# tech-srl/code2vec

Measured on NVIDIA H100. Metric: path-contexts/sec (train step, batch 1024x200), higher is better.
Workload: dtype tf32 operands / fp32 accumulate+storage

## Files before the change

### code2vec_b200/csrc/engine.cu

```cuda
#include <cuda_runtime.h>
#include <math.h>
#include <stdio.h>
#include <stdlib.h>
#include <string.h>

#include <string>
#include <utility>
#include <vector>

#include "../../include/c2v_b200.h"
#include "common.cuh"
#include "kernels.cuh"
#include "sgemm.cuh"
#include "umma_gemm.cuh"

using namespace c2v;

namespace {

thread_local std::string g_create_error = "";

constexpr size_t kAlign = 256;
inline size_t align_up(size_t x, size_t a = kAlign) { return (x + a - 1) / a * a; }

// ... 1 lines not shown
constexpr int kSplitDw = 48;

struct Workspace {
  size_t H, Xg, dXg, alpha, v, dv, S, loss_b, lse, loss, part, da_part, lse_part, dl;
  size_t Xg_lo, H_lo, S_lo, tgt_hi, tgt_lo, W_hi, W_lo, v_hi, v_lo;
  size_t WT, WT_lo, vT, vT_lo, tgtT, tgtT_lo;
  size_t true_logit, rscale, v_scaled, slab_flag;
  size_t st_src, st_pth, st_tgt, st_mask, st_target, st_topk_idx, st_topk_val, st_code, st_attn;
  size_t nx_src, nx_pth, nx_tgt;
  size_t sb_src, sb_pth, sb_tgt, sb_mask, sb_target;
  size_t stamp_tok, stamp_path, last_tok, last_path, lr_tab;
  size_t stamp_tgt, last_tgt;
  size_t perm, bkt_count, bkt_cursor, bkt_starts;
  size_t det_keys[2], det_vals[2], det_hist, det_offs, det_starts, det_part;
  size_t samp_stamp, samp_status;
  size_t total;
  size_t ldS;
  size_t ldB;
};

bool dims_ok(const c2v_dims* d, std::string* why) {
  auto bad = [&](const char* m) { if (why) *why = m; return false; };
  if (!d) return bad("dims is NULL");
  if (d->token_vocab < 1 || d->path_vocab < 1 || d->target_vocab < 1) return bad("vocab sizes must be >= 1");
  if (d->embed_dim < 4 || d->embed_dim % 4) return bad("embed_dim must be a positive multiple of 4");
  if (d->code_dim < 4 || d->code_dim % 4 || d->code_dim > 1024) return bad("code_dim must be a multiple of 4 in [4, 1024]");
  if (d->max_contexts < 1) return bad("max_contexts must be >= 1");
  if (d->max_batch < 1) return bad("max_batch must be >= 1");
  if (d->top_k < 1 || d->top_k > 64) return bad("top_k must be in [1, 64]");
  if ((double)d->max_batch * d->max_contexts > 2.0e9) return bad("max_batch * max_contexts overflows int32");
// ... 8 lines not shown
  size_t off = 0;
  auto take = [&](size_t bytes) { size_t o = off; off = align_up(off + bytes); return o; };
  w.H = take(N * D * 4);
  w.Xg = take(N * X * 4);
  w.dXg = take(N * X * 4);
  w.alpha = take(N * 4);
  w.v = take(B * D * 4);
  w.dv = take(B * D * 4);
  w.S = take(B * w.ldS * 4);
  w.loss_b = take(B * 4);
  w.lse = take(B * 4);
  w.true_logit = take(B * 4);
  w.rscale = take(B * 4);
  w.v_scaled = take(B * D * 4);
  w.slab_flag = take(64);
  w.loss = take(64);
  size_t part = (size_t)kSplitDv * B * D;
  if ((size_t)kSplitDw * X * D > part) part = (size_t)kSplitDw * X * D;
  w.part = take(part * 4);
  w.da_part = take(B * D * 4);
  w.lse_part = take(B * (size_t)umma::lse_slots(d.target_vocab) * 8);
  w.dl = take(B * (size_t)(kMaxSampled + 1) * 4);
  w.st_src = take(N * 4);
  w.st_pth = take(N * 4);
  w.st_tgt = take(N * 4);
  w.st_mask = take(N * 4);
  w.nx_src = take(N * 4);
  w.nx_pth = take(N * 4);
  w.nx_tgt = take(N * 4);
  w.st_target = take(B * 4);
// ... 114 lines not shown
  int sort_peer = 1;
  bool bkt_zeroed = false;
  int recompute = 0;
  int exp_slab = 1;
  bool slab_flag_zeroed = false;
  HeadSchedule split_fwd = HEAD_SIMT;
  int gather_occ[2] = {0, 0};
  int adam_epi_prefetch = 0;
  int fuse_sg = 0;
  int fuse_gather = 0;
  int cta_pair = 2;
  int num_sms;
  cudaEvent_t ev_tgt_ready = nullptr;
  int dy_late = 1;
  PendingDy pending_dy;
  cudaStream_t side = nullptr;
  cudaEvent_t ev_fork = nullptr, ev_join = nullptr;
  cudaStream_t copy = nullptr;
  cudaEvent_t ev_h2d[2] = {nullptr, nullptr}, ev_used[2] = {nullptr, nullptr};
  bool used_valid[2] = {false, false};
  uint64_t async_n = 0;
  cudaStream_t side2 = nullptr;
  cudaEvent_t ev_fork2 = nullptr, ev_join2 = nullptr;
  bool dy_in_flight = false;
  bool tgt_armed = false;
  float tgt_lr = 0.f, tgt_b1 = 0.f, tgt_b2 = 0.f, tgt_eps = 0.f;
  int64_t tgt_t = 0;
  int64_t armed_t = 0;
  const int32_t* hint_src = nullptr;
  const int32_t* hint_pth = nullptr;
// ... 679 lines not shown
  else
    C2V_LAUNCH(e, (topk_iter_kernel<<<Bt, kTopkThreads, 0, st>>>(S, e->ws.ldS, Y, k, 0, idx, val, row0)));
  if (stats) C2V_LAUNCH(e, (row_maxsum_kernel<<<Bt, 256, 0, st>>>(nullptr, 0, S, e->ws.ldS, Y, nullptr, 0, row_max, row_sum, nullptr)));
  return C2V_OK;
}

int run_dy(c2v_engine* e, cudaStream_t st, const float* v, int B, const SlabDesc& slab);

int run_pending_dy(c2v_engine* e, cudaStream_t st) {
  if (!e->pending_dy.v) return C2V_OK;
  const PendingDy p = e->pending_dy;
  e->pending_dy = PendingDy{};
  return run_dy(e, st, p.v, p.B, p.slab);
}

int context_backward(c2v_engine* e, cudaStream_t st, const ContextSource& cs, const float* mask, int B,
                     const Dropout& dp, const float* dv) {
  const int D = e->dims.code_dim, d = e->dims.embed_dim, K3 = 3 * d, N = cs.rows;
  float* H = wsp<float>(e, e->ws.H);
  float* alpha = wsp<float>(e, e->ws.alpha);
  float* da_part = wsp<float>(e, e->ws.da_part);
  float* part = wsp<float>(e, e->ws.part);
  int rc;
  if (ordered_route(e) && e->inbox.world < 2)
    return fail(e, C2V_ERR_STATE, "ordered_exchange: the gradient rows of row-sharded tables travel through the scatter inbox, "
                                  "and none is bound (c2v_bind_scatter_inbox)");
  if (!is_tc(e) && (rc = run_pending_dy(e, st))) return rc;
  const bool x3 = is_tc(e) && is_3x(e);
  float* H_lo = x3 ? wsp<float>(e, e->ws.H_lo) : nullptr;
  rc = launch_attn_bwd(e, st, H, alpha, dv, wsp<float>(e, e->ws.v), B, da_part, H_lo);
  if (rc) return rc;
  rc = launch_colsum(e, st, da_part, (size_t)D, B, D, e->grad.a);
  if (rc) return rc;
  if (is_tc(e)) {
    float* Xg = wsp<float>(e, e->ws.Xg);
    float* dXg = wsp<float>(e, e->ws.dXg);
    {
      PhaseTimer pt(e, PH_DX_GEMM, st);
      umma::Operand opA{H, (size_t)D, false, H_lo};
      umma::Operand opB{x3 ? wsp<float>(e, e->ws.W_hi) : e->theta.W, (size_t)D, false, x3 ? wsp<float>(e, e->ws.W_lo) : nullptr};
      umma::EpiStore ep{dXg, (size_t)K3, 0};
      C2V_LAUNCH(e, C2V_CUDA(e, (umma::launch(st, N, K3, D, 1, opA, opB, ep, e->num_sms))));
    }
    if (e->lazy) {
      if (e->lazy_grads_pending)
        return fail(e, C2V_ERR_STATE, "lazy_adam: every train step must be followed by c2v_adam_step before the next one");
      e->lazy_grads_pending = true;
    } else if (!e->emb_grads_clean && e->table_world == 1) {
      C2V_CUDA(e, cudaMemsetAsync(e->grad.tok, 0, (size_t)e->dims.token_vocab * d * 4, st));
      C2V_CUDA(e, cudaMemsetAsync(e->grad.path, 0, (size_t)e->dims.path_vocab * d * 4, st));
    }
    C2V_CUDA(e, cudaEventRecord(e->ev_fork, st));
    C2V_CUDA(e, cudaStreamWaitEvent(e->side, e->ev_fork, 0));
    {
      PhaseTimer pt(e, PH_DX_SCATTER, e->side);
      BucketPlan bp;
      if (ordered_route(e)) {
        e->sorted_src = nullptr;
        if ((rc = exchange_scatter(e, e->side, cs, mask, dp, dXg, false))) return rc;
      } else if (e->inbox.world > 1 && plan_buckets(e, &bp, true)) {
        if (e->sorted_src != cs.src || e->sorted_rows != cs.rows) {
          if ((rc = sort_entries(e, e->side, cs, bp))) return rc;
        }
        e->sorted_src = nullptr;
        const int32_t* starts = wsp<int32_t>(e, e->ws.bkt_starts);
        C2V_LAUNCH(e, (inbox_counts_kernel<<<1, 32, 0, e->side>>>(e->inbox, bp, starts)));
        C2V_LAUNCH(e, (scatter_inbox_kernel<<<(3 * N + 7) / 8, 256, 0, e->side>>>(cs, dp, mask, wsp<int32_t>(e, e->ws.perm), starts, bp, dXg,
                                                                              e->inbox, e->grad_scale)));
      } else if (plan_buckets(e, &bp)) {
        if ((rc = sort_entries(e, e->side, cs, bp))) return rc;
        C2V_LAUNCH(e, (scatter_sorted_kernel<<<(3 * N + 7) / 8, 256, 0, e->side>>>(cs, dp, mask, wsp<int32_t>(e, e->ws.perm), dXg, e->gr_tok,
                                                                               e->gr_path, e->grad_scale)));
      } else if (e->deterministic) {
        if ((rc = det_scatter(e, e->side, cs, mask, dp, dXg, false))) return rc;
      } else {
        C2V_LAUNCH(e, (scatter_dx_kernel<<<(N + 7) / 8, 256, 0, e->side>>>(cs, dp, mask, dXg, e->gr_tok, e->gr_path, e->grad_scale)));
      }
    }
    if ((rc = early_catchup(e, e->side))) return rc;
    C2V_CUDA(e, cudaEventRecord(e->ev_join, e->side));
    if ((rc = run_pending_dy(e, st))) return rc;
    {
      PhaseTimer pt(e, PH_DW, st);
      umma::Operand opA{Xg, (size_t)K3, true, x3 ? wsp<float>(e, e->ws.Xg_lo) : nullptr};
      umma::Operand opB{H, (size_t)D, true, H_lo};
      const int ks = umma::effective_splits(N, kSplitDw);
      umma::EpiStore ep{part, (size_t)D, (size_t)K3 * D};
      C2V_LAUNCH(e, C2V_CUDA(e, (umma::launch(st, K3, D, N, kSplitDw, opA, opB, ep, e->num_sms))));
      rc = launch_colsum(e, st, part, (size_t)K3 * D, ks, K3 * D, e->grad.W);
      if (rc) return rc;
    }
    C2V_CUDA(e, cudaStreamWaitEvent(st, e->ev_join, 0));
    if (e->dy_in_flight) {
      C2V_CUDA(e, cudaStreamWaitEvent(st, e->ev_join2, 0));
      e->dy_in_flight = false;
    }
    e->emb_grads_clean = false;
    return C2V_OK;
  }
  {
    PhaseTimer pt(e, PH_DW, st);
    simt::GatherColsX al{cs, dp};
    simt::ColsX bl{H, (size_t)D};
    const int ks = simt::effective_ksplit(N, kSplitDw);
    simt::StoreC ep{part, (size_t)D, (size_t)K3 * D};
    C2V_LAUNCH(e, C2V_CUDA(e, simt::launch(st, K3, D, N, kSplitDw, al, bl, ep)));
    rc = launch_colsum(e, st, part, (size_t)K3 * D, ks, K3 * D, e->grad.W);
// ... 239 lines not shown
      if ((rc = slab_to_p(e, st, hs, v, B, g, &slab, &v_dy))) return rc;
      C2V_LAUNCH(e, (loss_reduce_kernel<<<1, 256, 0, st>>>(loss_b, B, invB, loss_out)));
    }
  } else {
    if ((rc = run_logits(e, st, v, B, hs == HEAD_SIMT ? LOGITS_STORE : LOGITS_STORE_LSE, {}, true))) return rc;
    PhaseTimer pt(e, PH_XENT, st);
    if (hs == HEAD_SIMT) {
      C2V_LAUNCH(e, (xent_kernel<<<B, kXentThreads, 0, st>>>(S, e->ws.ldS, target, Y, invB, loss_b, lse, 1)));
    } else {
      C2V_LAUNCH(e, (xent_combine_kernel<<<B, 256, 0, st>>>(part, n_tiles, S, e->ws.ldS, target, loss_b, lse)));
      if ((rc = slab_to_p(e, st, hs, v, B, g, &slab, &v_dy))) return rc;
    }
    C2V_LAUNCH(e, (loss_reduce_kernel<<<1, 256, 0, st>>>(loss_b, B, invB, loss_out)));
  }
  if ((rc = target_grad_gemms(e, st, v_dy, B, dv, slab))) return rc;
  return context_backward(e, st, cs, mask, B, dp, dv);
}

int sampled_train_step_impl(c2v_engine* e, cudaStream_t st, const int32_t* src, const int32_t* pth, const int32_t* tgt,
                             const float* mask, const int32_t* target, int B, const int32_t* sampled, int S,
                             const float* logq_true, const float* logq_samp, float keep, uint64_t seed, uint64_t step,
                             const float* ext_mask, float* loss_out) {
  if (!e->has_grad) return fail(e, C2V_ERR_STATE, "gradients not bound (c2v_bind_grads)");
  if (!(keep > 0.f) || keep > 1.f) return fail(e, C2V_ERR_INVALID, "keep_prob must be in (0, 1]");
  if (S < 1 || S > kMaxSampled) return fail(e, C2V_ERR_INVALID, "number of sampled classes must be in [1, 1024]");
  const int D = e->dims.code_dim;
  const Dropout dp = make_dropout(e->dims, keep, seed, step, ext_mask);
  ContextSource cs = make_source(e, src, pth, tgt, B);
  float* H = wsp<float>(e, e->ws.H);
  float* alpha = wsp<float>(e, e->ws.alpha);
  float* v = wsp<float>(e, e->ws.v);
// ... 270 lines not shown
    if (value && !exchange_keys_fit(e->dims))
      return fail(e, C2V_ERR_UNSUPPORTED, "ordered_exchange: the padded rows of both tables over all ranks must be below 2^31");
    e->ordered_exchange = (int)value;
    return C2V_OK;
  }
  if (!strcmp(key, "profile")) { e->profile = value ? 1 : 0; return C2V_OK; }
  if (!strcmp(key, "dy_late")) {
    if (value < 0 || value > 2) return fail(e, C2V_ERR_INVALID, "dy_late must be 0, 1 or 2");
    e->dy_late = (int)value;
    return C2V_OK;
  }
  if (!strcmp(key, "fuse_target_adam")) { e->fuse_tgt = value ? 1 : 0; return C2V_OK; }
  if (!strcmp(key, "fuse_gather")) { e->fuse_gather = value ? 1 : 0; return C2V_OK; }
  if (!strcmp(key, "fuse_softmax_grad")) { e->fuse_sg = value ? 1 : 0; return C2V_OK; }
  if (!strcmp(key, "exp_slab")) { e->exp_slab = value ? 1 : 0; return C2V_OK; }
  if (!strcmp(key, "adam_epilogue_prefetch")) { e->adam_epi_prefetch = value ? 1 : 0; return C2V_OK; }
  if (!strcmp(key, "recompute_logits")) { e->recompute = value ? 1 : 0; return C2V_OK; }
  if (!strcmp(key, "sort_peer_access")) {
    if (value < 0 || value > 2) return fail(e, C2V_ERR_INVALID, "sort_peer_access must be 0 (never), 1 (auto) or 2 (always)");
    e->sort_peer = (int)value;
    return C2V_OK;
  }
  if (!strcmp(key, "adam_rest_shortcut")) { e->rest_shortcut = value ? 1 : 0; return C2V_OK; }
  if (!strcmp(key, "adam_sweep_period")) {
    if (value < 0 || value > kLrRing / 2) return fail(e, C2V_ERR_INVALID, "adam_sweep_period must be in [0, 32768]");
    e->sweep_period = (int)value;
    return C2V_OK;
  }
  if (!strcmp(key, "adam_rows_occupancy")) {
    if (value != 4 && value != 5) return fail(e, C2V_ERR_INVALID, "adam_rows_occupancy must be 4 or 5");
// ... 80 lines not shown
        return C2V_ERR_CUDA;
      *value = n;
    }
    return C2V_OK;
  }
  if (!strcmp(key, "profile")) { *value = e->profile; return C2V_OK; }
  if (!strcmp(key, "lazy_adam")) { *value = e->lazy; return C2V_OK; }
  if (!strcmp(key, "adam_sweep_period")) { *value = e->sweep_period; return C2V_OK; }
  if (!strcmp(key, "adam_rest_shortcut")) { *value = e->rest_shortcut; return C2V_OK; }
  if (!strcmp(key, "cta_pair")) { *value = e->cta_pair; return C2V_OK; }
  if (!strcmp(key, "dy_late")) { *value = e->dy_late; return C2V_OK; }
  if (!strcmp(key, "fuse_target_adam")) { *value = e->fuse_tgt; return C2V_OK; }
  if (!strcmp(key, "fuse_gather")) { *value = e->fuse_gather; return C2V_OK; }
  if (!strcmp(key, "fuse_softmax_grad")) { *value = e->fuse_sg; return C2V_OK; }
  if (!strcmp(key, "exp_slab")) { *value = e->exp_slab; return C2V_OK; }
  if (!strcmp(key, "adam_epilogue_prefetch")) { *value = e->adam_epi_prefetch; return C2V_OK; }
  if (!strcmp(key, "exp_slab_fallbacks")) {
    *value = 0;
    if (e->wbase && e->slab_flag_zeroed) {
      unsigned n = 0;
      if (cudaDeviceSynchronize() != cudaSuccess ||
          cudaMemcpy(&n, e->wbase + e->ws.slab_flag + 4, 4, cudaMemcpyDeviceToHost) != cudaSuccess)
        return C2V_ERR_CUDA;
      *value = n;
    }
    return C2V_OK;
  }
  if (!strcmp(key, "sampler_cap_hits")) {
    *value = 0;
    if (e->wbase && e->sample_tag) {
// ... 602 lines not shown
  if (!ordered_route(e)) return fail(e, C2V_ERR_STATE, "set ordered_exchange and bind row-sharded tables over more than one rank first");
  if (e->inbox.world < 2) return fail(e, C2V_ERR_STATE, "no scatter inbox bound (c2v_bind_scatter_inbox)");
  if ((int64_t)n_tok + n_path > 3ll * e->dims.max_batch * e->dims.max_contexts)
    return fail(e, C2V_ERR_INVALID, "n_tok + n_path must be at most 3 * max_batch * max_contexts");
  if (((uintptr_t)tok_vals | (uintptr_t)path_vals) % 16) return fail(e, C2V_ERR_INVALID, "tok_vals and path_vals must be 16-byte aligned");
  C2V_CUDA(e, cudaSetDevice(e->device));
  cudaStream_t st = (cudaStream_t)stream;
  const size_t d = (size_t)e->dims.embed_dim;
  float* vals = wsp<float>(e, e->ws.dXg);
  if (n_tok) C2V_CUDA(e, cudaMemcpyAsync(vals, tok_vals, n_tok * d * 4, cudaMemcpyDeviceToDevice, st));
  if (n_path) C2V_CUDA(e, cudaMemcpyAsync(vals + n_tok * d, path_vals, n_path * d * 4, cudaMemcpyDeviceToDevice, st));
  return exchange_push(e, st, ExchangeListKeys{tok_rows, path_rows, n_tok, exchange_key_map(e)}, n_tok + n_path,
                       DetListContrib{vals, (int)d});
}

int64_t c2v_launch_count(const c2v_engine* e) { return e ? e->launches : 0; }

int c2v_phase_count(void) { return PH_COUNT; }

const char* c2v_phase_name(int phase) { return (phase >= 0 && phase < PH_COUNT) ? kPhaseNames[phase] : ""; }

int c2v_phase_stats(c2v_engine* e, int phase, double* total_ms, int64_t* count, int reset) {
  if (!e || phase < 0 || phase >= PH_COUNT) return C2V_ERR_INVALID;
  C2V_CUDA(e, cudaSetDevice(e->device));
  PhaseLog& L = e->phase[phase];
  if (!L.pending.empty()) C2V_CUDA(e, cudaDeviceSynchronize());
  for (auto& ev : L.pending) {
    float ms = 0.f;
    if (cudaEventElapsedTime(&ms, ev.first, ev.second) == cudaSuccess) { L.total_ms += ms; L.count++; }
    L.free_list.push_back(ev);
// ... 10 lines not shown
```

### code2vec_b200/csrc/kernels.cuh

```cuda
#pragma once
#include <float.h>
#include <limits.h>
#include "common.cuh"

namespace c2v {

constexpr int kAttnThreads = 128;
constexpr int kAttnWarps = kAttnThreads / 32;

__device__ __forceinline__ float block_sum(float v, float* red) {
  const int lane = threadIdx.x & 31, warp = threadIdx.x >> 5, nw = (blockDim.x + 31) >> 5;
  v = warp_sum(v);
  __syncthreads();
  if (lane == 0) red[warp] = v;
  __syncthreads();
  float r = (threadIdx.x < nw) ? red[threadIdx.x] : 0.f;
  if (warp == 0) {
    r = warp_sum(r);
    if (lane == 0) red[0] = r;
  }
  __syncthreads();
  r = red[0];
  __syncthreads();
  return r;
// ... 917 lines not shown
  if (mask[n] == 0.f) return;
  const int K3 = 3 * cs.d;
  const float* src = dXg + (size_t)n * K3;
  for (int j = lane * 4; j < K3; j += 128) {
    float4 g = *reinterpret_cast<const float4*>(src + j);
    const float4 m = dropout_mult4(dp, n, j >> 2);
    g.x *= m.x * grad_scale; g.y *= m.y * grad_scale; g.z *= m.z * grad_scale; g.w *= m.w * grad_scale;
    const int seg = j / cs.d, off = j - seg * cs.d;
    float* dst;
    if (seg == 0) dst = table_row(g_tok, cs.src[n], cs.d) + off;
    else if (seg == 1) dst = table_row(g_path, cs.pth[n], cs.d) + off;
    else dst = table_row(g_tok, cs.tgt[n], cs.d) + off;
    atomicAdd(reinterpret_cast<float4*>(dst), g);
  }
}

constexpr int kMaxBuckets = 8192;

struct BucketPlan {
  int shift, mask;
  int page_shift;
  int pages_tok, pages_path;
  int n_buckets;
};
__device__ __forceinline__ int bucket_of(const BucketPlan& bp, int seg, int idx) {
  const int owner = idx & bp.mask, page = (idx >> bp.shift) >> bp.page_shift;
  return (seg == 1) ? (bp.mask + 1) * bp.pages_tok + owner * bp.pages_path + page : owner * bp.pages_tok + page;
}
__device__ __forceinline__ int entry_index(const ContextSource& cs, int e) {
  const int n = e / 3, seg = e - 3 * n;
// ... 722 lines not shown
```

### code2vec_b200/csrc/umma_gemm.cuh

```cuda
#pragma once
#include <cuda.h>
#include <cuda_runtime.h>
#include <limits.h>
#include <stdint.h>

#include "common.cuh"

namespace c2v {
namespace umma {

constexpr int BM = 128;
constexpr int BN = 128;
constexpr int BK = 32;
constexpr int WG_K = 8;
constexpr int STAGES = 4;
constexpr int kThreads = 4 * 128;
constexpr int kRegsProducer = 72;
constexpr int kRegsConsumer = 128;
constexpr int kRegsEpilogue = 184;
static_assert(kRegsProducer + 2 * kRegsConsumer + kRegsEpilogue == 4 * 128, "the roles share the CTA's registers");

__device__ __forceinline__ float fast_tanh(float x) {
  float e, r;
  asm("ex2.approx.ftz.f32 %0, %1;" : "=f"(e) : "f"(x * 2.885390081777927f));
// ... 8 lines not shown
}
__device__ __forceinline__ void mbar_expect_tx(uint64_t* bar, uint32_t bytes) {
  asm volatile("mbarrier.expect_tx.relaxed.cta.shared::cta.b64 [%0], %1;" ::"r"(smem_u32(bar)), "r"(bytes) : "memory");
}
__device__ __forceinline__ void mbar_arrive(uint64_t* bar) {
  asm volatile("mbarrier.arrive.shared::cta.b64 _, [%0];" ::"r"(smem_u32(bar)) : "memory");
}
__device__ __forceinline__ void mbar_arrive_expect_tx(uint64_t* bar, uint32_t bytes) {
  asm volatile("mbarrier.arrive.expect_tx.shared::cta.b64 _, [%0], %1;" ::"r"(smem_u32(bar)), "r"(bytes) : "memory");
}
__device__ __forceinline__ bool mbar_try_wait(uint64_t* bar, uint32_t parity) {
  uint32_t ok;
  asm volatile(
      "{\n\t.reg .pred p;\n\t"
      "mbarrier.try_wait.parity.shared::cta.b64 p, [%1], %2;\n\t"
      "selp.u32 %0, 1, 0, p;\n\t}"
      : "=r"(ok) : "r"(smem_u32(bar)), "r"(parity) : "memory");
  return ok != 0;
}
template <bool SLEEP = false>
__device__ __forceinline__ void mbar_wait(uint64_t* bar, uint32_t parity) {
  if (mbar_try_wait(bar, parity)) return;
  const long long t0 = clock64();
  uint32_t ns = 32;
  while (!mbar_try_wait(bar, parity)) {
    if (SLEEP) {
      __nanosleep(ns);
      if (ns < 256) ns *= 2;
    }
    if (clock64() - t0 > 20000000000LL) __trap();
// ... 611 lines not shown
  size_t lda;
};

struct SmemLayout {
  static constexpr int kABytes = BM * BK * 4;
  static constexpr int kBBytes = BN * BK * 4;
  static constexpr int kStageBytes = kABytes + kBBytes;
  static constexpr int kEpiOffset = STAGES * kStageBytes;
  static constexpr int kEpiBytes = 64 * BN * 4;
  static constexpr int kBarOffset = kEpiOffset + 2 * kEpiBytes;
  static constexpr int kTotal = kBarOffset + 256 + 1024;
  static_assert((3 * STAGES + 2) * 8 <= 256, "the barriers fit their block");
  static_assert(kTotal <= 232448, "exceeds the 227 KB of shared memory a CTA can opt into");
};

template <bool A_MN, bool B_MN, class Epi, class AX = AXNone, bool B_T = false>
__global__ void __launch_bounds__(kThreads, 1)
umma_gemm_kernel(const __grid_constant__ CUtensorMap tmA, const __grid_constant__ CUtensorMap tmB,
                 const __grid_constant__ CUtensorMap tmAlo, const __grid_constant__ CUtensorMap tmBlo, GemmShape gs,
                 GemmPtrs ptr, Epi epi, AX ax = AX{}, BTransposed bt = {}) {
  if (epi_gate_closed(epi, 0)) return;
  using L = SmemLayout;
  static_assert(!(A_MN && AX::kKind == 2), "the gathered A tile is K-major");
  constexpr bool kTmaA = !A_MN && AX::kKind == 0;
  constexpr bool kTmaB = !B_MN;
  static_assert(!B_T || (kTmaA && kTmaB), "the B tile is copied out of all-K-major TMA stages");
  constexpr uint32_t kTxBytes = (kTmaA ? L::kABytes : 0) + (kTmaB ? L::kBBytes : 0);
  constexpr uint32_t kMnTxBytes = (A_MN ? L::kABytes : 0) + (B_MN ? L::kBBytes : 0);
  constexpr int kLag = kMnTxBytes ? STAGES - 2 : 0;
  static_assert(kLag <= STAGES - 2, "the producer would wait for a stage only a step it has not published can free");
  extern __shared__ uint8_t smem_raw[];
  uint8_t* smem = reinterpret_cast<uint8_t*>((reinterpret_cast<uintptr_t>(smem_raw) + 1023) & ~(uintptr_t)1023);
  uint64_t* full_bar = reinterpret_cast<uint64_t*>(smem + L::kBarOffset);
  uint64_t* empty_bar = full_bar + STAGES;
  uint64_t* landed_bar = empty_bar + STAGES;
// ... 174 lines not shown
    if constexpr (epi_move_regs<Epi>(0)) wg_regs_inc<kRegsEpilogue>();
    const int w = warp & 3;
    float* stg = reinterpret_cast<float*>(smem + L::kEpiOffset + (w >> 1) * L::kEpiBytes);
    auto prefetch_item = [&](int it) {
      if (it >= total_items) return;
      int mt2, nt2, sp2;
      decode(it, mt2, nt2, sp2);
      epi_prefetch_tile(epi, mt2 * BM + 32 * w + lane, nt2 * BN, BN, gs.M, gs.N, 0);
    };
    prefetch_item(blockIdx.x);
    uint32_t epi_phase = 0;
    for (int item = blockIdx.x; item < total_items; item += gridDim.x, epi_phase ^= 1) {
      int mt, nt, sp;
      decode(item, mt, nt, sp);
      prefetch_item(item + gridDim.x);
      mbar_wait<true>(epi_full, epi_phase);
      const int m_base = mt * BM + 32 * w, m = m_base + lane;
      float* cbase = epi.out(sp);
#pragma unroll 1
      for (int p = 0; p < 2; ++p) {
        typename Epi::State est;
        epi.begin(est);
#pragma unroll 1
        for (int q = p; q < 4; q += 2) {
          float* blk = stg + ((w & 1) | (q << 1)) * 1024;
          uint32_t r[32];
#pragma unroll
          for (int c4 = 0; c4 < 8; ++c4) {
            const float4 x = *reinterpret_cast<const float4*>(blk + lane * 32 + ((c4 ^ (lane & 7)) << 2));
            r[4 * c4] = __float_as_uint(x.x); r[4 * c4 + 1] = __float_as_uint(x.y);
            r[4 * c4 + 2] = __float_as_uint(x.z); r[4 * c4 + 3] = __float_as_uint(x.w);
          }
          __syncwarp();
          const int n = nt * BN + 32 * q;
          if (n < gs.N) {
            if (m < gs.M) epi.observe(m, n, r, gs.N - n, est);
            if (epi_stores<Epi>(0)) store_chunk(epi, est, r, blk, lane, m_base, n, gs.M, gs.N, cbase, epi.ldc);
          }
        }
        epi.end(m, 2 * nt + p, sp, m < gs.M, est);
      }
      mbar_arrive(epi_empty);
    }
  }
}

typedef CUresult (*EncodeTiledFn)(CUtensorMap*, CUtensorMapDataType, cuuint32_t, void*, const cuuint64_t*, const cuuint64_t*,
                                  const cuuint32_t*, const cuuint32_t*, CUtensorMapInterleave, CUtensorMapSwizzle,
                                  CUtensorMapL2promotion, CUtensorMapFloatOOBfill);

inline EncodeTiledFn get_encode_fn() {
  static EncodeTiledFn fn = nullptr;
  if (!fn) {
    void* p = nullptr;
    cudaDriverEntryPointQueryResult qres;
    if (cudaGetDriverEntryPoint("cuTensorMapEncodeTiled", &p, cudaEnableDefault, &qres) == cudaSuccess && p)
      fn = reinterpret_cast<EncodeTiledFn>(p);
// ... 50 lines not shown
inline GemmShape make_shape(int M, int N, int K, int splits, int terms) {
  GemmShape gs;
  gs.M = M; gs.N = N; gs.K = K;
  gs.terms = terms;
  gs.m_tiles = (M + BM - 1) / BM;
  gs.n_tiles = (N + BN - 1) / BN;
  const int total_kblocks = (K + BK - 1) / BK;
  if (splits < 1) splits = 1;
  if (splits > total_kblocks) splits = total_kblocks;
  gs.kblocks_per_split = (total_kblocks + splits - 1) / splits;
  gs.splits = (total_kblocks + gs.kblocks_per_split - 1) / gs.kblocks_per_split;
  gs.n_fastest = (gs.n_tiles < gs.m_tiles) ? 1 : 0;
  return gs;
}

template <bool A_MN, bool B_MN, class Epi, class AX, bool B_T = false>
inline cudaError_t launch_kernel(cudaStream_t st, const CUtensorMap& tmA, const CUtensorMap& tmB, const CUtensorMap& tmAlo,
                                 const CUtensorMap& tmBlo, const GemmShape& gs, const GemmPtrs& ptr, const Epi& epi, int num_sms,
                                 const AX& ax, const BTransposed& bt = {}) {
  auto kern = umma_gemm_kernel<A_MN, B_MN, Epi, AX, B_T>;
  cudaError_t e = cudaFuncSetAttribute(kern, cudaFuncAttributeMaxDynamicSharedMemorySize, SmemLayout::kTotal);
  if (e != cudaSuccess) return e;
  int grid = gs.m_tiles * gs.n_tiles * gs.splits;
  if (grid > num_sms) grid = num_sms;
  kern<<<grid, kThreads, SmemLayout::kTotal, st>>>(tmA, tmB, tmAlo, tmBlo, gs, ptr, epi, ax, bt);
  return cudaGetLastError();
}

template <bool A_MN, bool B_MN, class Epi, class AX = AXNone, bool B_T = false>
inline cudaError_t launch_cfg(cudaStream_t st, int M, int N, int K, int splits, const Operand& A, const Operand& B, const Epi& epi,
                              int num_sms, const AX& ax = AX{}, const BTransposed& bt = {}) {
  CUtensorMap tmA{}, tmB{}, tmAlo{}, tmBlo{};
  const bool three = A.lo != nullptr && B.lo != nullptr;
  if ((A.lo != nullptr) != (B.lo != nullptr)) return cudaErrorInvalidValue;
  if (AX::kKind != 0 && three) return cudaErrorInvalidValue;
  if (B_T && (!bt.hi || (three && !bt.lo) || bt.ld < (size_t)N || bt.ld % 4 || K % 4 ||
              ((reinterpret_cast<uintptr_t>(bt.hi) | reinterpret_cast<uintptr_t>(bt.lo)) % 16)))
    return cudaErrorInvalidValue;
  if (A_MN || AX::kKind == 0) {
    if (!operand_map(&tmA, A.base, A_MN, M, K, A.ld)) return cudaErrorInvalidValue;
    if (three && !operand_map(&tmAlo, A.lo, A_MN, M, K, A.ld)) return cudaErrorInvalidValue;
  }
  if (!operand_map(&tmB, B.base, B_MN, N, K, B.ld)) return cudaErrorInvalidValue;
  if (three && !operand_map(&tmBlo, B.lo, B_MN, N, K, B.ld)) return cudaErrorInvalidValue;
  const GemmPtrs ptr{A.base, A.ld};
  return launch_kernel<A_MN, B_MN, Epi, AX, B_T>(st, tmA, tmB, tmAlo, tmBlo, make_shape(M, N, K, splits, three ? 3 : 1), ptr, epi,
                                                 num_sms, ax, bt);
}

inline int effective_splits(int K, int splits) {
  const int total_kblocks = (K + BK - 1) / BK;
  if (splits < 1) splits = 1;
  if (splits > total_kblocks) splits = total_kblocks;
  const int per = (total_kblocks + splits - 1) / splits;
  return (total_kblocks + per - 1) / per;
}

inline int lse_slots(int n) { return 2 * ((n + BN - 1) / BN); }

template <class Epi>
inline cudaError_t launch(cudaStream_t st, int M, int N, int K, int splits, const Operand& A, const Operand& B, const Epi& epi,
                          int num_sms) {
// ... 25 lines not shown
```

### code2vec_b200/engine.py

```python
from __future__ import annotations

import ctypes as C
import os
from dataclasses import dataclass
from typing import Dict, Optional, Tuple

import numpy as np

from . import build as _build

PARAM_NAMES = ("tok", "path", "tgt", "W", "a")

MATH_FP32 = 0
MATH_TF32 = 1
MATH_3XTF32 = 2
MATH_MODES = {"fp32": MATH_FP32, "tf32": MATH_TF32, "3xtf32": MATH_3XTF32}


class c2v_dims(C.Structure):
    _fields_ = [(n, C.c_int32) for n in ("token_vocab", "path_vocab", "target_vocab", "embed_dim",
                                         "code_dim", "max_contexts", "max_batch", "top_k")]


class c2v_tensors(C.Structure):
# ... 64 lines not shown
                                       C.c_float, C.c_float, C.c_float, C.c_float, _P, _P]),
    "c2v_train_batch_async": (C.c_int, [_P, _P, _P, _P, _P, _P, _I32, C.c_float, C.c_uint64, C.c_int64,
                                        C.c_float, C.c_float, C.c_float, C.c_float, _P, _P, _P]),
    "c2v_predict_batch_host": (C.c_int, [_P, _P, _P, _P, _P, _I32, _I32, _P, _P, _P, _P, _P]),
    "c2v_selftest_gemm": (C.c_int, [_P, _I32, _I32, _I32, _I32, _I32, _I32, _I32, _P, C.c_size_t, _P, C.c_size_t,
                                    _P, C.c_size_t, _P]),
    "c2v_selftest_gemm3": (C.c_int, [_P, _I32, _I32, _I32, _I32, _I32, _I32, _I32, _P, _P, C.c_size_t, _P, _P, C.c_size_t,
                                     _P, C.c_size_t, _P]),
    "c2v_selftest_gemm_bt": (C.c_int, [_P, _I32, _I32, _I32, _P, C.c_size_t, _P, C.c_size_t, _P, C.c_size_t, _P, C.c_size_t,
                                       _P]),
    "c2v_selftest_split": (C.c_int, [_P, _P, _P, _P, C.c_size_t, _P]),
    "c2v_selftest_transpose": (C.c_int, [_P, _P, _I32, _I32, _P, _P, C.c_size_t, _P]),
    "c2v_selftest_target_t": (C.c_int, [_P, _I32, C.POINTER(C.c_size_t), C.POINTER(C.c_size_t)]),
    "c2v_selftest_row_sum": (C.c_int, [_P, _I32, _P, _P, _I32, _P, _P]),
    "c2v_selftest_exchange_push": (C.c_int, [_P, _P, _P, _I32, _P, _P, _I32, _P]),
    "c2v_set_event": (C.c_int, [_P, C.c_char_p, _P]),
    "c2v_sync_tables": (C.c_int, [_P, _P]),
    "c2v_context_forward": (C.c_int, [_P, _P, _P, _P, _P, _I32, C.c_float, C.c_uint64, C.c_uint64, _P, _P, _P]),
    "c2v_target_forward": (C.c_int, [_P, _P, _I32, _P, _I32, _P, _P, _P, _P]),
    "c2v_lse_combine": (C.c_int, [_P, _P, _P, _I32, _I32, _P, C.c_float, _P, _P, _P]),
    "c2v_target_backward": (C.c_int, [_P, _P, _I32, _P, _P, _I32, C.c_float, _P, _P]),
    "c2v_context_backward": (C.c_int, [_P, _P, _P, _P, _P, _I32, C.c_float, C.c_uint64, C.c_uint64, _P, _P, _P]),
    "c2v_topk_partial": (C.c_int, [_P, _P, _I32, _I32, _I32, _P, _P, _P, _P, _P]),
    "c2v_topk_merge": (C.c_int, [_P, _P, _P, _P, _P, _I32, _I32, _I32, _I32, _I32, _I32, _P, _P, _P]),
    "c2v_launch_count": (C.c_int64, [_P]),
    "c2v_phase_count": (C.c_int, []),
    "c2v_phase_name": (C.c_char_p, [C.c_int]),
    "c2v_phase_stats": (C.c_int, [_P, C.c_int, C.POINTER(C.c_double), C.POINTER(C.c_int64), C.c_int]),
    "c2v_reader_create": (C.c_int, [_I32, C.POINTER(c2v_reader_vocab), C.POINTER(c2v_reader_vocab),
                                    C.POINTER(c2v_reader_vocab), C.c_int, C.POINTER(_P)]),
# ... 357 lines not shown

    def loss(self, code_vec, target):
        out = self.torch.empty(1, dtype=self.torch.float32, device=self.dev)
        self._check(self.lib.c2v_loss(self.h, code_vec.data_ptr(), target.data_ptr(), code_vec.shape[0],
                                      out.data_ptr(), self._stream()))
        return out

    def train_step(self, src, path, tgt, mask, target, keep: float = 1.0, seed: int = 0, step: int = 0,
                   dropout_mask=None, loss_out=None):
        out = self._loss if loss_out is None else loss_out
        self._check(self.lib.c2v_train_step(self.h, src.data_ptr(), path.data_ptr(), tgt.data_ptr(), mask.data_ptr(),
                                            target.data_ptr(), src.shape[0], float(keep), int(seed), int(step),
                                            _ptr(dropout_mask), out.data_ptr(), self._stream()))
        return out

    def sampled_train_step(self, src, path, tgt, mask, target, sampled, logq_true, logq_sampled, keep: float = 1.0,
                           seed: int = 0, step: int = 0, dropout_mask=None, loss_out=None):
        out = self._loss if loss_out is None else loss_out
        self._check(self.lib.c2v_sampled_train_step(
            self.h, src.data_ptr(), path.data_ptr(), tgt.data_ptr(), mask.data_ptr(), target.data_ptr(),
            src.shape[0], sampled.data_ptr(), sampled.shape[0], logq_true.data_ptr(), logq_sampled.data_ptr(),
            float(keep), int(seed), int(step), _ptr(dropout_mask), out.data_ptr(), self._stream()))
        return out

    def sample_log_uniform(self, target, S: int, seed: int, step: int):
        torch = self.torch
        B, S = int(target.shape[0]), int(S)
        buf = getattr(self, "_sampler_out", None)
        if buf is None:
            z = lambda n, dt: torch.empty(n, dtype=dt, device=self.dev)
# ... 221 lines not shown
```

### include/c2v_b200.h

```cpp
#ifndef C2V_B200_H_
#define C2V_B200_H_

#include <stddef.h>
#include <stdint.h>

#ifdef __cplusplus
extern "C" {
#endif

#define C2V_ABI_VERSION 1

typedef struct c2v_engine c2v_engine;

typedef enum c2v_status {
  C2V_OK = 0,
  C2V_ERR_INVALID = -1,
  C2V_ERR_CUDA = -2,
  C2V_ERR_STATE = -3,
  C2V_ERR_UNSUPPORTED = -4
} c2v_status;

typedef struct c2v_dims {
  int32_t token_vocab;
  int32_t path_vocab;
// ... 143 lines not shown

int c2v_selftest_gemm_bt(c2v_engine* e, int32_t M, int32_t N, int32_t K, const float* A, size_t lda, const float* B,
                         size_t ldb, float* C, size_t ldc, float* BT, size_t ldbt, void* stream);

int c2v_selftest_transpose(c2v_engine* e, const float* x, int32_t rows, int32_t cols, float* xT, float* xT_lo, size_t ldT,
                           void* stream);

int c2v_selftest_target_t(const c2v_engine* e, int32_t lo, size_t* offset, size_t* ld);

int c2v_selftest_row_sum(c2v_engine* e, int32_t table_id, const int32_t* rows, const float* vals, int32_t count,
                         float* out, void* stream);

int c2v_selftest_exchange_push(c2v_engine* e, const int32_t* tok_rows, const float* tok_vals, int32_t n_tok,
                               const int32_t* path_rows, const float* path_vals, int32_t n_path, void* stream);

int64_t c2v_launch_count(const c2v_engine* e);

int c2v_phase_count(void);
const char* c2v_phase_name(int phase);
int c2v_phase_stats(c2v_engine* e, int phase, double* total_ms, int64_t* count, int reset);

typedef struct c2v_reader c2v_reader;

typedef struct c2v_reader_vocab {
  const void* slots;
  const char* bytes;
  uint64_t mask;
  int32_t oov;
  int32_t pad;
} c2v_reader_vocab;
// ... 139 lines not shown
```

Measured before the change: 32.14 million.

## Fuse embedding-gradient scatter into dW GEMM epilogue warps as co-work

The dW split-K GEMM kernel gains an optional CoWork hook. Its epilogue warps, while waiting on the accumulator barrier and after their tiles finish, pull chunks of contexts from a global atomic counter and scatter dXg rows into the token and path gradient tables with atomicAdd. This replaces the separate scatter kernel on a side stream and its fork and join. The aim is to fill idle epilogue time and drop a launch and the stream synchronization. The cost is memory traffic and atomic contention inside the GEMM, which could slow the tensor-core mainloop, and the grid is now always sized to the SM count.

After: 32.36 million (median of 6 runs). Within noise of the previous version (+0.7%).

```diff
diff --git a/code2vec_b200/csrc/engine.cu b/code2vec_b200/csrc/engine.cu
--- a/code2vec_b200/csrc/engine.cu
+++ b/code2vec_b200/csrc/engine.cu
@@ -39,6 +39,7 @@
   size_t perm, bkt_count, bkt_cursor, bkt_starts;
   size_t det_keys[2], det_vals[2], det_hist, det_offs, det_starts, det_part;
   size_t samp_stamp, samp_status;
+  size_t cowork_next;
   size_t total;
   size_t ldS;
   size_t ldB;
@@ -77,6 +78,7 @@
   w.rscale = take(B * 4);
   w.v_scaled = take(B * D * 4);
   w.slab_flag = take(64);
+  w.cowork_next = take(64);
   w.loss = take(64);
   size_t part = (size_t)kSplitDv * B * D;
   if ((size_t)kSplitDw * X * D > part) part = (size_t)kSplitDw * X * D;
@@ -221,6 +223,7 @@
   cudaEvent_t ev_tgt_ready = nullptr;
   int dy_late = 1;
   PendingDy pending_dy;
+  int dw_cowork = 1;
   cudaStream_t side = nullptr;
   cudaEvent_t ev_fork = nullptr, ev_join = nullptr;
   cudaStream_t copy = nullptr;
@@ -930,8 +933,74 @@
   return run_dy(e, st, p.v, p.B, p.slab);
 }
 
+int run_dw(c2v_engine* e, cudaStream_t st, const ContextSource& cs, const float* mask, const Dropout& dp, bool cowork) {
+  const int D = e->dims.code_dim, K3 = 3 * e->dims.embed_dim, N = cs.rows;
+  const bool x3 = is_3x(e);
+  float* H = wsp<float>(e, e->ws.H);
+  float* part = wsp<float>(e, e->ws.part);
+  PhaseTimer pt(e, PH_DW, st);
+  umma::Operand opA{wsp<float>(e, e->ws.Xg), (size_t)K3, true, x3 ? wsp<float>(e, e->ws.Xg_lo) : nullptr};
+  umma::Operand opB{H, (size_t)D, true, x3 ? wsp<float>(e, e->ws.H_lo) : nullptr};
+  const int ks = umma::effective_splits(N, kSplitDw);
+  umma::EpiStore ep{part, (size_t)D, (size_t)K3 * D};
+  if (cowork) {
+    int* next = wsp<int>(e, e->ws.cowork_next);
+    C2V_CUDA(e, cudaMemsetAsync(next, 0, sizeof(int), st));
+    const DxScatterCoWork cw{cs, dp, mask, wsp<float>(e, e->ws.dXg), e->gr_tok, e->gr_path, e->grad_scale, next};
+    C2V_LAUNCH(e, C2V_CUDA(e, (umma::launch_cfg<true, true, umma::EpiStore, umma::AXNone, false, DxScatterCoWork>(
+                                  st, K3, D, N, kSplitDw, opA, opB, ep, e->num_sms, {}, {}, cw))));
+  } else {
+    C2V_LAUNCH(e, C2V_CUDA(e, (umma::launch(st, K3, D, N, kSplitDw, opA, opB, ep, e->num_sms))));
+  }
+  return launch_colsum(e, st, part, (size_t)K3 * D, ks, K3 * D, e->grad.W);
+}
+
+int scatter_and_dw(c2v_engine* e, cudaStream_t st, const ContextSource& cs, const float* mask, const Dropout& dp, bool cowork) {
+  int rc;
+  if (cowork) {
+    if ((rc = run_pending_dy(e, st))) return rc;
+    if ((rc = run_dw(e, st, cs, mask, dp, true))) return rc;
+    return early_catchup(e, st);
+  }
+  const int N = cs.rows;
+  float* dXg = wsp<float>(e, e->ws.dXg);
+  C2V_CUDA(e, cudaEventRecord(e->ev_fork, st));
+  C2V_CUDA(e, cudaStreamWaitEvent(e->side, e->ev_fork, 0));
+  {
+    PhaseTimer pt(e, PH_DX_SCATTER, e->side);
+    BucketPlan bp;
+    if (ordered_route(e)) {
+      e->sorted_src = nullptr;
+      if ((rc = exchange_scatter(e, e->side, cs, mask, dp, dXg, false))) return rc;
+    } else if (e->inbox.world > 1 && plan_buckets(e, &bp, true)) {
+      if (e->sorted_src != cs.src || e->sorted_rows != cs.rows) {
+        if ((rc = sort_entries(e, e->side, cs, bp))) return rc;
+      }
+      e->sorted_src = nullptr;
+      const int32_t* starts = wsp<int32_t>(e, e->ws.bkt_starts);
+      C2V_LAUNCH(e, (inbox_counts_kernel<<<1, 32, 0, e->side>>>(e->inbox, bp, starts)));
+      C2V_LAUNCH(e, (scatter_inbox_kernel<<<(3 * N + 7) / 8, 256, 0, e->side>>>(cs, dp, mask, wsp<int32_t>(e, e->ws.perm), starts, bp, dXg,
+                                                                            e->inbox, e->grad_scale)));
+    } else if (plan_buckets(e, &bp)) {
+      if ((rc = sort_entries(e, e->side, cs, bp))) return rc;
+      C2V_LAUNCH(e, (scatter_sorted_kernel<<<(3 * N + 7) / 8, 256, 0, e->side>>>(cs, dp, mask, wsp<int32_t>(e, e->ws.perm), dXg, e->gr_tok,
+                                                                             e->gr_path, e->grad_scale)));
+    } else if (e->deterministic) {
+      if ((rc = det_scatter(e, e->side, cs, mask, dp, dXg, false))) return rc;
+    } else {
+      C2V_LAUNCH(e, (scatter_dx_kernel<<<(N + 7) / 8, 256, 0, e->side>>>(cs, dp, mask, dXg, e->gr_tok, e->gr_path, e->grad_scale)));
+    }
+  }
+  if ((rc = early_catchup(e, e->side))) return rc;
+  C2V_CUDA(e, cudaEventRecord(e->ev_join, e->side));
+  if ((rc = run_pending_dy(e, st))) return rc;
+  if ((rc = run_dw(e, st, cs, mask, dp, false))) return rc;
+  C2V_CUDA(e, cudaStreamWaitEvent(st, e->ev_join, 0));
+  return C2V_OK;
+}
+
 int context_backward(c2v_engine* e, cudaStream_t st, const ContextSource& cs, const float* mask, int B,
-                     const Dropout& dp, const float* dv) {
+                     const Dropout& dp, const float* dv, bool cowork_ok = false) {
   const int D = e->dims.code_dim, d = e->dims.embed_dim, K3 = 3 * d, N = cs.rows;
   float* H = wsp<float>(e, e->ws.H);
   float* alpha = wsp<float>(e, e->ws.alpha);
@@ -949,7 +1018,6 @@
   rc = launch_colsum(e, st, da_part, (size_t)D, B, D, e->grad.a);
   if (rc) return rc;
   if (is_tc(e)) {
-    float* Xg = wsp<float>(e, e->ws.Xg);
     float* dXg = wsp<float>(e, e->ws.dXg);
     {
       PhaseTimer pt(e, PH_DX_GEMM, st);
@@ -966,47 +1034,8 @@
       C2V_CUDA(e, cudaMemsetAsync(e->grad.tok, 0, (size_t)e->dims.token_vocab * d * 4, st));
       C2V_CUDA(e, cudaMemsetAsync(e->grad.path, 0, (size_t)e->dims.path_vocab * d * 4, st));
     }
-    C2V_CUDA(e, cudaEventRecord(e->ev_fork, st));
-    C2V_CUDA(e, cudaStreamWaitEvent(e->side, e->ev_fork, 0));
-    {
-      PhaseTimer pt(e, PH_DX_SCATTER, e->side);
-      BucketPlan bp;
-      if (ordered_route(e)) {
-        e->sorted_src = nullptr;
-        if ((rc = exchange_scatter(e, e->side, cs, mask, dp, dXg, false))) return rc;
-      } else if (e->inbox.world > 1 && plan_buckets(e, &bp, true)) {
-        if (e->sorted_src != cs.src || e->sorted_rows != cs.rows) {
-          if ((rc = sort_entries(e, e->side, cs, bp))) return rc;
-        }
-        e->sorted_src = nullptr;
-        const int32_t* starts = wsp<int32_t>(e, e->ws.bkt_starts);
-        C2V_LAUNCH(e, (inbox_counts_kernel<<<1, 32, 0, e->side>>>(e->inbox, bp, starts)));
-        C2V_LAUNCH(e, (scatter_inbox_kernel<<<(3 * N + 7) / 8, 256, 0, e->side>>>(cs, dp, mask, wsp<int32_t>(e, e->ws.perm), starts, bp, dXg,
-                                                                              e->inbox, e->grad_scale)));
-      } else if (plan_buckets(e, &bp)) {
-        if ((rc = sort_entries(e, e->side, cs, bp))) return rc;
-        C2V_LAUNCH(e, (scatter_sorted_kernel<<<(3 * N + 7) / 8, 256, 0, e->side>>>(cs, dp, mask, wsp<int32_t>(e, e->ws.perm), dXg, e->gr_tok,
-                                                                               e->gr_path, e->grad_scale)));
-      } else if (e->deterministic) {
-        if ((rc = det_scatter(e, e->side, cs, mask, dp, dXg, false))) return rc;
-      } else {
-        C2V_LAUNCH(e, (scatter_dx_kernel<<<(N + 7) / 8, 256, 0, e->side>>>(cs, dp, mask, dXg, e->gr_tok, e->gr_path, e->grad_scale)));
-      }
-    }
-    if ((rc = early_catchup(e, e->side))) return rc;
-    C2V_CUDA(e, cudaEventRecord(e->ev_join, e->side));
-    if ((rc = run_pending_dy(e, st))) return rc;
-    {
-      PhaseTimer pt(e, PH_DW, st);
-      umma::Operand opA{Xg, (size_t)K3, true, x3 ? wsp<float>(e, e->ws.Xg_lo) : nullptr};
-      umma::Operand opB{H, (size_t)D, true, H_lo};
-      const int ks = umma::effective_splits(N, kSplitDw);
-      umma::EpiStore ep{part, (size_t)D, (size_t)K3 * D};
-      C2V_LAUNCH(e, C2V_CUDA(e, (umma::launch(st, K3, D, N, kSplitDw, opA, opB, ep, e->num_sms))));
-      rc = launch_colsum(e, st, part, (size_t)K3 * D, ks, K3 * D, e->grad.W);
-      if (rc) return rc;
-    }
-    C2V_CUDA(e, cudaStreamWaitEvent(st, e->ev_join, 0));
+    if ((rc = scatter_and_dw(e, st, cs, mask, dp, cowork_ok && e->dw_cowork && e->table_world == 1 && !e->deterministic)))
+      return rc;
     if (e->dy_in_flight) {
       C2V_CUDA(e, cudaStreamWaitEvent(st, e->ev_join2, 0));
       e->dy_in_flight = false;
@@ -1276,7 +1305,7 @@
     C2V_LAUNCH(e, (loss_reduce_kernel<<<1, 256, 0, st>>>(loss_b, B, invB, loss_out)));
   }
   if ((rc = target_grad_gemms(e, st, v_dy, B, dv, slab))) return rc;
-  return context_backward(e, st, cs, mask, B, dp, dv);
+  return context_backward(e, st, cs, mask, B, dp, dv, true);
 }
 
 int sampled_train_step_impl(c2v_engine* e, cudaStream_t st, const int32_t* src, const int32_t* pth, const int32_t* tgt,
@@ -1577,6 +1606,7 @@
   if (!strcmp(key, "fuse_gather")) { e->fuse_gather = value ? 1 : 0; return C2V_OK; }
   if (!strcmp(key, "fuse_softmax_grad")) { e->fuse_sg = value ? 1 : 0; return C2V_OK; }
   if (!strcmp(key, "exp_slab")) { e->exp_slab = value ? 1 : 0; return C2V_OK; }
+  if (!strcmp(key, "dw_scatter_cowork")) { e->dw_cowork = value ? 1 : 0; return C2V_OK; }
   if (!strcmp(key, "adam_epilogue_prefetch")) { e->adam_epi_prefetch = value ? 1 : 0; return C2V_OK; }
   if (!strcmp(key, "recompute_logits")) { e->recompute = value ? 1 : 0; return C2V_OK; }
   if (!strcmp(key, "sort_peer_access")) {
@@ -1687,6 +1717,7 @@
   if (!strcmp(key, "fuse_gather")) { *value = e->fuse_gather; return C2V_OK; }
   if (!strcmp(key, "fuse_softmax_grad")) { *value = e->fuse_sg; return C2V_OK; }
   if (!strcmp(key, "exp_slab")) { *value = e->exp_slab; return C2V_OK; }
+  if (!strcmp(key, "dw_scatter_cowork")) { *value = e->dw_cowork; return C2V_OK; }
   if (!strcmp(key, "adam_epilogue_prefetch")) { *value = e->adam_epi_prefetch; return C2V_OK; }
   if (!strcmp(key, "exp_slab_fallbacks")) {
     *value = 0;
@@ -2319,6 +2350,34 @@
                        DetListContrib{vals, (int)d});
 }
 
+int c2v_selftest_dw_scatter(c2v_engine* e, int32_t route, const int32_t* src, const int32_t* path, const int32_t* tgt,
+                            const float* mask, int32_t B, float keep_prob, uint64_t seed, uint64_t step, void* stream) {
+  int rc = check_batch(e, B);
+  if (rc) return rc;
+  if (route < 0 || route > 3) return fail(e, C2V_ERR_INVALID, "route must be 0 (dW), 1 (scatter), 2 (fork / join) or 3 (co-work)");
+  if (!src || !path || !tgt || !mask) return fail(e, C2V_ERR_INVALID, "NULL argument");
+  if (!e->has_grad) return fail(e, C2V_ERR_STATE, "gradients not bound (c2v_bind_grads)");
+  if (!is_tc(e) || e->table_world != 1 || e->deterministic)
+    return fail(e, C2V_ERR_STATE, "needs a tensor-core math mode, tables that are not row-sharded and deterministic off");
+  C2V_CUDA(e, cudaSetDevice(e->device));
+  cudaStream_t st = (cudaStream_t)stream;
+  const Dropout dp = make_dropout(e->dims, keep_prob, seed, step, nullptr);
+  const ContextSource cs = make_source(e, src, path, tgt, B);
+  if (route == 0) return run_dw(e, st, cs, mask, dp, 0);
+  if (route == 1) {
+    C2V_LAUNCH(e, (scatter_dx_kernel<<<(cs.rows + 7) / 8, 256, 0, st>>>(cs, dp, mask, wsp<float>(e, e->ws.dXg), e->gr_tok, e->gr_path,
+                                                                       e->grad_scale)));
+    return C2V_OK;
+  }
+  return scatter_and_dw(e, st, cs, mask, dp, route == 3);
+}
+
+int c2v_selftest_dx_offset(const c2v_engine* e, size_t* offset) {
+  if (!e || !offset) return C2V_ERR_INVALID;
+  *offset = e->ws.dXg;
+  return C2V_OK;
+}
+
 int64_t c2v_launch_count(const c2v_engine* e) { return e ? e->launches : 0; }
 
 int c2v_phase_count(void) { return PH_COUNT; }
diff --git a/code2vec_b200/csrc/kernels.cuh b/code2vec_b200/csrc/kernels.cuh
--- a/code2vec_b200/csrc/kernels.cuh
+++ b/code2vec_b200/csrc/kernels.cuh
@@ -955,6 +955,64 @@
     atomicAdd(reinterpret_cast<float4*>(dst), g);
   }
 }
+
+struct DxScatterCoWork {
+  static constexpr bool kActive = true;
+  static constexpr int kCtx = 4;
+  static constexpr int kBatch = 12;
+  ContextSource cs;
+  Dropout dp;
+  const float* mask;
+  const float* dXg;
+  ShardedTable g_tok, g_path;
+  float grad_scale;
+  int* next;
+  __device__ __forceinline__ bool chunk(int lane) const {
+    int n0 = 0;
+    if (lane == 0) n0 = atomicAdd(next, kCtx);
+    n0 = __shfl_sync(0xffffffffu, n0, 0);
+    if (n0 >= cs.rows) return false;
+    int i_src = 0, i_pth = 0, i_tgt = 0;
+    bool ok = false;
+    if (lane < kCtx && n0 + lane < cs.rows) {
+      ok = mask[n0 + lane] != 0.f;
+      i_src = cs.src[n0 + lane]; i_pth = cs.pth[n0 + lane]; i_tgt = cs.tgt[n0 + lane];
+    }
+    const unsigned live = __ballot_sync(0xffffffffu, ok);
+    const int K3 = 3 * cs.d, q = K3 / 4, per = (q + 31) / 32;
+    const float* base = dXg + (size_t)n0 * K3;
+    for (int s0 = 0; s0 < kCtx * per; s0 += kBatch) {
+      float4 g[kBatch];
+      int c = s0 / per, k = s0 - c * per;
+#pragma unroll
+      for (int u = 0; u < kBatch; ++u) {
+        const int j4 = 32 * k + lane;
+        if (c < kCtx && ((live >> c) & 1) && j4 < q) g[u] = __ldcs(reinterpret_cast<const float4*>(base + (size_t)c * K3) + j4);
+        if (++k == per) { k = 0; ++c; }
+      }
+      c = s0 / per; k = s0 - c * per;
+#pragma unroll
+      for (int u = 0; u < kBatch; ++u) {
+        const int j4 = 32 * k + lane;
+        const int r_src = __shfl_sync(0xffffffffu, i_src, c & 31), r_pth = __shfl_sync(0xffffffffu, i_pth, c & 31),
+                  r_tgt = __shfl_sync(0xffffffffu, i_tgt, c & 31);
+        if (c < kCtx && ((live >> c) & 1) && j4 < q) {
+          const int n = n0 + c, j = 4 * j4;
+          const float4 m = dropout_mult4(dp, n, j4);
+          g[u].x *= m.x * grad_scale; g[u].y *= m.y * grad_scale; g[u].z *= m.z * grad_scale; g[u].w *= m.w * grad_scale;
+          const int seg = j < cs.d ? 0 : (j < 2 * cs.d ? 1 : 2), off = j - seg * cs.d;
+          float* dst;
+          if (seg == 0) dst = table_row(g_tok, r_src, cs.d) + off;
+          else if (seg == 1) dst = table_row(g_path, r_pth, cs.d) + off;
+          else dst = table_row(g_tok, r_tgt, cs.d) + off;
+          atomicAdd(reinterpret_cast<float4*>(dst), g[u]);
+        }
+        if (++k == per) { k = 0; ++c; }
+      }
+    }
+    return true;
+  }
+};
 
 constexpr int kMaxBuckets = 8192;
 
diff --git a/code2vec_b200/csrc/umma_gemm.cuh b/code2vec_b200/csrc/umma_gemm.cuh
--- a/code2vec_b200/csrc/umma_gemm.cuh
+++ b/code2vec_b200/csrc/umma_gemm.cuh
@@ -46,6 +46,15 @@
   asm volatile(
       "{\n\t.reg .pred p;\n\t"
       "mbarrier.try_wait.parity.shared::cta.b64 p, [%1], %2;\n\t"
+      "selp.u32 %0, 1, 0, p;\n\t}"
+      : "=r"(ok) : "r"(smem_u32(bar)), "r"(parity) : "memory");
+  return ok != 0;
+}
+__device__ __forceinline__ bool mbar_test_wait(uint64_t* bar, uint32_t parity) {
+  uint32_t ok;
+  asm volatile(
+      "{\n\t.reg .pred p;\n\t"
+      "mbarrier.test_wait.parity.shared::cta.b64 p, [%1], %2;\n\t"
       "selp.u32 %0, 1, 0, p;\n\t}"
       : "=r"(ok) : "r"(smem_u32(bar)), "r"(parity) : "memory");
   return ok != 0;
@@ -687,11 +696,16 @@
   static_assert(kTotal <= 232448, "exceeds the 227 KB of shared memory a CTA can opt into");
 };
 
-template <bool A_MN, bool B_MN, class Epi, class AX = AXNone, bool B_T = false>
+struct NoCoWork {
+  static constexpr bool kActive = false;
+  __device__ __forceinline__ bool chunk(int) const { return false; }
+};
+
+template <bool A_MN, bool B_MN, class Epi, class AX = AXNone, bool B_T = false, class CoWork = NoCoWork>
 __global__ void __launch_bounds__(kThreads, 1)
 umma_gemm_kernel(const __grid_constant__ CUtensorMap tmA, const __grid_constant__ CUtensorMap tmB,
                  const __grid_constant__ CUtensorMap tmAlo, const __grid_constant__ CUtensorMap tmBlo, GemmShape gs,
-                 GemmPtrs ptr, Epi epi, AX ax = AX{}, BTransposed bt = {}) {
+                 GemmPtrs ptr, Epi epi, AX ax = AX{}, BTransposed bt = {}, CoWork cw = {}) {
   if (epi_gate_closed(epi, 0)) return;
   using L = SmemLayout;
   static_assert(!(A_MN && AX::kKind == 2), "the gathered A tile is K-major");
@@ -896,6 +910,9 @@
       int mt, nt, sp;
       decode(item, mt, nt, sp);
       prefetch_item(item + gridDim.x);
+      if constexpr (CoWork::kActive) {
+        for (bool more = true; more && !__all_sync(0xffffffffu, mbar_test_wait(epi_full, epi_phase));) more = cw.chunk(lane);
+      }
       mbar_wait<true>(epi_full, epi_phase);
       const int m_base = mt * BM + 32 * w, m = m_base + lane;
       float* cbase = epi.out(sp);
@@ -923,6 +940,9 @@
         epi.end(m, 2 * nt + p, sp, m < gs.M, est);
       }
       mbar_arrive(epi_empty);
+    }
+    if constexpr (CoWork::kActive) {
+      while (cw.chunk(lane)) {}
     }
   }
 }
@@ -1003,22 +1023,22 @@
   return gs;
 }
 
-template <bool A_MN, bool B_MN, class Epi, class AX, bool B_T = false>
+template <bool A_MN, bool B_MN, class Epi, class AX, bool B_T = false, class CoWork = NoCoWork>
 inline cudaError_t launch_kernel(cudaStream_t st, const CUtensorMap& tmA, const CUtensorMap& tmB, const CUtensorMap& tmAlo,
                                  const CUtensorMap& tmBlo, const GemmShape& gs, const GemmPtrs& ptr, const Epi& epi, int num_sms,
-                                 const AX& ax, const BTransposed& bt = {}) {
-  auto kern = umma_gemm_kernel<A_MN, B_MN, Epi, AX, B_T>;
+                                 const AX& ax, const BTransposed& bt = {}, const CoWork& cw = {}) {
+  auto kern = umma_gemm_kernel<A_MN, B_MN, Epi, AX, B_T, CoWork>;
   cudaError_t e = cudaFuncSetAttribute(kern, cudaFuncAttributeMaxDynamicSharedMemorySize, SmemLayout::kTotal);
   if (e != cudaSuccess) return e;
   int grid = gs.m_tiles * gs.n_tiles * gs.splits;
-  if (grid > num_sms) grid = num_sms;
-  kern<<<grid, kThreads, SmemLayout::kTotal, st>>>(tmA, tmB, tmAlo, tmBlo, gs, ptr, epi, ax, bt);
+  if (grid > num_sms || CoWork::kActive) grid = num_sms;
+  kern<<<grid, kThreads, SmemLayout::kTotal, st>>>(tmA, tmB, tmAlo, tmBlo, gs, ptr, epi, ax, bt, cw);
   return cudaGetLastError();
 }
 
-template <bool A_MN, bool B_MN, class Epi, class AX = AXNone, bool B_T = false>
+template <bool A_MN, bool B_MN, class Epi, class AX = AXNone, bool B_T = false, class CoWork = NoCoWork>
 inline cudaError_t launch_cfg(cudaStream_t st, int M, int N, int K, int splits, const Operand& A, const Operand& B, const Epi& epi,
-                              int num_sms, const AX& ax = AX{}, const BTransposed& bt = {}) {
+                              int num_sms, const AX& ax = AX{}, const BTransposed& bt = {}, const CoWork& cw = {}) {
   CUtensorMap tmA{}, tmB{}, tmAlo{}, tmBlo{};
   const bool three = A.lo != nullptr && B.lo != nullptr;
   if ((A.lo != nullptr) != (B.lo != nullptr)) return cudaErrorInvalidValue;
@@ -1033,8 +1053,8 @@
   if (!operand_map(&tmB, B.base, B_MN, N, K, B.ld)) return cudaErrorInvalidValue;
   if (three && !operand_map(&tmBlo, B.lo, B_MN, N, K, B.ld)) return cudaErrorInvalidValue;
   const GemmPtrs ptr{A.base, A.ld};
-  return launch_kernel<A_MN, B_MN, Epi, AX, B_T>(st, tmA, tmB, tmAlo, tmBlo, make_shape(M, N, K, splits, three ? 3 : 1), ptr, epi,
-                                                 num_sms, ax, bt);
+  return launch_kernel<A_MN, B_MN, Epi, AX, B_T, CoWork>(st, tmA, tmB, tmAlo, tmBlo, make_shape(M, N, K, splits, three ? 3 : 1), ptr,
+                                                         epi, num_sms, ax, bt, cw);
 }
 
 inline int effective_splits(int K, int splits) {
diff --git a/code2vec_b200/engine.py b/code2vec_b200/engine.py
--- a/code2vec_b200/engine.py
+++ b/code2vec_b200/engine.py
@@ -102,6 +102,8 @@
     "c2v_selftest_target_t": (C.c_int, [_P, _I32, C.POINTER(C.c_size_t), C.POINTER(C.c_size_t)]),
     "c2v_selftest_row_sum": (C.c_int, [_P, _I32, _P, _P, _I32, _P, _P]),
     "c2v_selftest_exchange_push": (C.c_int, [_P, _P, _P, _I32, _P, _P, _I32, _P]),
+    "c2v_selftest_dw_scatter": (C.c_int, [_P, _I32, _P, _P, _P, _P, _I32, C.c_float, C.c_uint64, C.c_uint64, _P]),
+    "c2v_selftest_dx_offset": (C.c_int, [_P, C.POINTER(C.c_size_t)]),
     "c2v_set_event": (C.c_int, [_P, C.c_char_p, _P]),
     "c2v_sync_tables": (C.c_int, [_P, _P]),
     "c2v_context_forward": (C.c_int, [_P, _P, _P, _P, _P, _I32, C.c_float, C.c_uint64, C.c_uint64, _P, _P, _P]),
@@ -489,6 +491,17 @@
                                             _ptr(dropout_mask), out.data_ptr(), self._stream()))
         return out
 
+    def selftest_dw_scatter(self, route: int, src, path, tgt, mask, keep: float = 1.0, seed: int = 0, step: int = 0):
+        self._check(self.lib.c2v_selftest_dw_scatter(self.h, int(route), src.data_ptr(), path.data_ptr(), tgt.data_ptr(),
+                                                     mask.data_ptr(), src.shape[0], float(keep), int(seed), int(step),
+                                                     self._stream()))
+
+    def selftest_dx(self, rows: int):
+        off = C.c_size_t()
+        self._check(self.lib.c2v_selftest_dx_offset(self.h, C.byref(off)))
+        n = rows * 3 * self.dims.embed_dim
+        return self.workspace[off.value:off.value + 4 * n].view(self.torch.float32).view(rows, 3 * self.dims.embed_dim)
+
     def sampled_train_step(self, src, path, tgt, mask, target, sampled, logq_true, logq_sampled, keep: float = 1.0,
                            seed: int = 0, step: int = 0, dropout_mask=None, loss_out=None):
         out = self._loss if loss_out is None else loss_out
diff --git a/include/c2v_b200.h b/include/c2v_b200.h
--- a/include/c2v_b200.h
+++ b/include/c2v_b200.h
@@ -181,6 +181,11 @@
 int c2v_selftest_exchange_push(c2v_engine* e, const int32_t* tok_rows, const float* tok_vals, int32_t n_tok,
                                const int32_t* path_rows, const float* path_vals, int32_t n_path, void* stream);
 
+int c2v_selftest_dw_scatter(c2v_engine* e, int32_t route, const int32_t* src, const int32_t* path, const int32_t* tgt,
+                            const float* mask, int32_t B, float keep_prob, uint64_t seed, uint64_t step, void* stream);
+
+int c2v_selftest_dx_offset(const c2v_engine* e, size_t* offset);
+
 int64_t c2v_launch_count(const c2v_engine* e);
 
 int c2v_phase_count(void);
```
